# wyhuai/DDNM

Hardware: AMD Instinct MI355X
Metric: restored images/sec @256×256, 100 DDIM steps, 4×SR; 1/2/4/8 GPU (higher is better)
Workload: dtype f32 (3x3 convolutions: fp32 operands carried as hi + lo fp16 halves, three fp16 MFMA products per product, fp32 accumulate -- operand error 2^-22, measured closer to fp64 than the fp32 MFMA kernel; everything else fp32); 1 GPU; celeba_hq.yml SVD sr_bicubic 4x, sigma_y=0, eta=0.85, T_sampling=100, batch_size=8 per GPU (BASELINE configs[1]); global_batch=8, image=3x256x256, parallelism=dp1 (image sharding)

## Files before the change

ddnm_amd/_lib.py:

```python
import ctypes
import os
from ctypes import POINTER, Structure, c_char_p, c_float, c_int32, c_int64, c_uint32, c_void_p

_HERE = os.path.dirname(os.path.abspath(__file__))
LIB_PATH = os.path.join(_HERE, "libddnm_hip.so")

c_f32p = c_void_p


class ConvDesc(Structure):
    _fields_ = [
        ("src0", c_void_p), ("src1", c_void_p), ("weight", c_void_p), ("bias", c_void_p),
        ("badd", c_void_p), ("res", c_void_p), ("gn_scale", c_void_p), ("gn_shift", c_void_p),
        ("out", c_void_p),
        ("B", c_int32), ("Hin", c_int32), ("Win", c_int32),
        ("C0", c_int32), ("C1", c_int32), ("Cout", c_int32),
        ("ksize", c_int32), ("stride", c_int32), ("pad", c_int32),
        ("Ho", c_int32), ("Wo", c_int32),
        ("ups", c_int32), ("gn_silu", c_int32), ("out_nchw", c_int32),
        ("badd_stride", c_int32), ("tile", c_int32),
        ("workspace", c_void_p), ("workspace_floats", c_int64),
        ("res_ups", c_int32), ("src_f16", c_int32),
        ("stats_out", c_void_p),
        ("skip0", c_void_p), ("skip1", c_void_p), ("skip_weight", c_void_p),
# ... 70 lines not shown
                                    c_int32, c_void_p]),
    "ddnm_gn_finalize_tiles_f32": (c_int32, [c_void_p, c_int32, c_int32, c_void_p, c_int32, c_int32, c_void_p, c_void_p,
                                             c_int32, c_int32, c_int32, c_float, c_void_p, c_void_p, c_void_p, c_int32,
                                             c_void_p, c_void_p]),
    "ddnm_gn_finalize_tiles_amax_f32": (c_int32, [c_void_p, c_int32, c_int32, c_void_p, c_int32, c_int32, c_void_p, c_void_p,
                                                  c_int32, c_int32, c_int32, c_float, c_void_p, c_void_p, c_void_p, c_int32,
                                                  c_void_p, c_void_p, c_void_p]),
    "ddnm_amax_bound_f32": (c_int32, [c_void_p, c_int64, c_int32, c_void_p, c_int64, c_int32, c_void_p, c_int32, c_void_p]),
    "ddnm_conv3x3_f16_f32": (c_int32, [POINTER(ConvDesc), c_void_p]),
    "ddnm_conv3x3_f16_supported": (c_int32, [POINTER(ConvDesc)]),
    "ddnm_conv3x3_f16_workspace_floats": (c_int64, [POINTER(ConvDesc)]),
    "ddnm_conv3x3_f16_stats_tiles": (c_int32, [POINTER(ConvDesc)]),
    "ddnm_conv3x3_s16_f32": (c_int32, [POINTER(ConvDesc), c_void_p]),
    "ddnm_conv3x3_s16_supported": (c_int32, [POINTER(ConvDesc)]),
    "ddnm_conv3x3_s16_persistent": (c_int32, [POINTER(ConvDesc)]),
    "ddnm_conv3x3_s16_ups_subpixel_supported": (c_int32, [POINTER(ConvDesc)]),
    "ddnm_conv3x3_s16_workspace_floats": (c_int64, [POINTER(ConvDesc)]),
    "ddnm_conv3x3_s16_stats_tiles": (c_int32, [POINTER(ConvDesc)]),
    "ddnm_conv3x3_s16_act_scale": (c_float, []),
    "ddnm_conv_gather_s16_f32": (c_int32, [POINTER(ConvDesc), c_void_p]),
    "ddnm_conv_gather_s16_supported": (c_int32, [POINTER(ConvDesc)]),
    "ddnm_conv_gather_s16_workspace_floats": (c_int64, [POINTER(ConvDesc)]),
    "ddnm_conv_gather_s16_stats_tiles": (c_int32, [POINTER(ConvDesc)]),
    "ddnm_conv16": (c_int32, [POINTER(Conv16Desc), c_void_p]),
    "ddnm_conv16_supported": (c_int32, [POINTER(Conv16Desc)]),
    "ddnm_conv16_fuses_fin": (c_int32, [POINTER(Conv16Desc)]),
    "ddnm_conv16_workspace_floats": (c_int64, [POINTER(Conv16Desc)]),
    "ddnm_conv16_stats_tiles": (c_int32, [POINTER(Conv16Desc)]),
    "ddnm_gn_apply_h16": (c_int32, [c_void_p, c_void_p, c_void_p, c_void_p, c_void_p, c_int32, c_int32, c_int32, c_int32,
                                    c_int32, c_int32, c_int32, c_void_p]),
    "ddnm_im2col3x3_h16": (c_int32, [c_void_p, c_void_p, c_void_p, c_void_p, c_void_p, c_int32, c_int32, c_int32, c_int32,
                                     c_int32, c_int32, c_void_p]),
    "ddnm_nchw_to_nhwc_h16": (c_int32, [c_void_p, c_void_p, c_int32, c_int32, c_int32, c_int32, c_void_p]),
    "ddnm_gn_stats_h16": (c_int32, [c_void_p, c_void_p, c_int32, c_int32, c_int32, c_int32, c_void_p]),
    "ddnm_attn16_d64": (c_int32, [c_void_p, c_void_p, c_int32, c_int32, c_int32, c_void_p]),
    "ddnm_conv1x1_f16_f32": (c_int32, [POINTER(ConvDesc), c_void_p]),
    "ddnm_conv1x1_f16_supported": (c_int32, [POINTER(ConvDesc)]),
    "ddnm_conv1x1_f16_workspace_floats": (c_int64, [POINTER(ConvDesc)]),
    "ddnm_conv1x1_f16_stats_tiles": (c_int32, [POINTER(ConvDesc)]),
    "ddnm_gn_stats_f32": (c_int32, [c_void_p, c_void_p, c_int32, c_int32, c_int32, c_int32, c_int32, c_void_p,
                                    c_int32, c_void_p]),
    "ddnm_gn_nchunk": (c_int32, [c_int32, c_int32]),
    "ddnm_gn_finalize_f32": (c_int32, [c_void_p, c_int32, c_void_p, c_void_p, c_int32, c_int32, c_int32, c_int32,
                                       c_float, c_void_p, c_void_p, c_void_p, c_int32, c_void_p, c_void_p]),
    "ddnm_bgemm_f32": (c_int32, [POINTER(GemmDesc), c_void_p]),
    "ddnm_gn_bwd_f32": (c_int32, [c_void_p, c_void_p, c_int32, c_void_p, c_void_p, c_void_p, c_int32, c_void_p, c_int32,
# ... 154 lines not shown
```

ddnm_amd/build.py:

```python
import hashlib
import os
import shutil
import subprocess
import sys

HERE = os.path.dirname(os.path.abspath(__file__))
CSRC = os.path.join(HERE, "csrc")
LIB = os.path.join(HERE, "libddnm_hip.so")
STAMP = os.path.join(HERE, ".libddnm_hip.stamp")
OBJ = os.path.join(HERE, "_obj")
SOURCES = ["conv_igemm_f32.hip", "conv_igemm_f16.hip", "conv_s16_persist.hip", "conv_s16_subpixel.hip", "conv_gather_s16.hip", "conv_small_f32.hip", "conv1x1_f16.hip", "conv16.hip", "act16.hip", "attn16.hip", "attn_d512.hip", "attn16_bwd.hip", "gemm_f32.hip", "groupnorm.hip", "misc.hip", "ddnm_step.hip", "fwht.hip", "backward.hip", "metrics.hip"]
FLAGS = ["--offload-arch=gfx950", "-O3", "-std=c++17", "-fPIC", "-shared", "-Wall", "-Wno-unused-function"]


def _hipcc():
    for c in (os.environ.get("HIPCC"), shutil.which("hipcc"), "/opt/rocm/bin/hipcc"):
        if c and os.path.exists(c):
            return c
    raise RuntimeError("hipcc not found (set HIPCC)")


def _digest():
    h = hashlib.sha256()
    for f in sorted(os.listdir(CSRC)) + ["../../include/ddnm_hip.h"]:
        with open(os.path.join(CSRC, f), "rb") as fh:
            h.update(f.encode() + fh.read())
    h.update(" ".join(FLAGS).encode())
    return h.hexdigest()


LAST_BUILD = {"compiled": False}


def build(force=False, verbose=False):
# ... 64 lines not shown
```

ddnm_amd/csrc/conv_s16_persist.hip:

```cpp
#include <type_traits>

#include "conv_common.h"

typedef unsigned u32x4 __attribute__((ext_vector_type(4)));

namespace {
constexpr int P_WM = 4, P_WN = 2, P_MT = 2, P_NT = 2;
constexpr int P_NTHREADS = 512, P_BN = 128;
constexpr int P_LDH = 72, P_KCH = 32;
constexpr int P_MAXH = 340, P_HWD = 34;
constexpr int P_HCOLS = 8, P_HRPP = P_NTHREADS / P_HCOLS, P_HR = (P_MAXH + P_HRPP - 1) / P_HRPP, P_HSPLIT = (P_HR + 1) / 2;
constexpr int P_BR = P_BN / (P_NTHREADS / 8);
constexpr int P_NWB = 3, P_WTILE = P_BN * 128;
constexpr int P_HBYTES = 2 * P_MAXH * P_LDH * 2;
constexpr int P_NOUT = P_MT * P_NT * 16;
enum { K_MID = 0, K_LAST = 1, K_FIRST = 2 };

constexpr int p_spread(int tap) { return tap == 0 ? 10 : (tap <= 6 ? 9 : 0); }
constexpr int p_first_of(int tap) { return tap == 0 ? 0 : (tap <= 7 ? 10 + 9 * (tap - 1) : P_NOUT); }
static_assert(p_first_of(7) == P_NOUT, "64 values over taps 0..6");
constexpr int p_extra(int kind, int tap, bool has_res, bool ascale) {
    return kind == K_FIRST ? p_spread(tap) + (tap == 0 ? 1 : 0)
                           : (kind == K_LAST ? (tap == 0 ? 4 + (ascale ? 1 : 0) : 0) + (has_res ? p_spread(tap) : 0) : 0);
}
// ... 440 lines not shown
        if (!have_next) break;
        v = vn;
        cur_base = next_base;
        cur_stats = next_stats;
        epi_cur = epi_next;
        pending = true;
    }
    __syncthreads();
    store_stats();
#pragma unroll
    for (int k = 0; k < P_NOUT; ++k) __builtin_amdgcn_raw_buffer_store_b32(__float_as_uint(outv[k]), r_out, o_lane, o_soff(pend_base, k), 0);
}

bool conv3x3_s16_persist_eligible(const ConvArgs& p) {
    const ddnm_conv_desc& d = p.d;
    const long tiles = (long)p.m_tiles * p.n_tiles;
    if (d.skip0 && (!d.amax_in || d.res)) return false;
    return p.ksplit == 1 && tiles >= 512 && p.TW == 32 && !d.res_ups && !d.out_nchw && p.Cin / P_KCH >= 2 &&
           (int64_t)d.B * d.Ho * d.Wo * d.Cout * 4 < ((int64_t)1 << 31) && (int64_t)p.m_tiles * d.Cout * 8 < ((int64_t)1 << 31);
}

int conv3x3_s16_persist_launch(const ConvArgs& p, hipStream_t s) {
    const int cus = conv_persist_grid_cus();
    const int total = p.m_tiles * p.n_tiles;
    const dim3 grid(total < cus ? total : cus);
    const bool asc = p.d.amax_in != nullptr, res = p.d.res != nullptr;
    if (p.d.skip0) { DDNM_LAUNCH((conv3x3_s16_persist_kernel<true, false, true>), grid, dim3(P_NTHREADS), 0, s, p, total); }
    else if (asc && res) { DDNM_LAUNCH((conv3x3_s16_persist_kernel<true, true>), grid, dim3(P_NTHREADS), 0, s, p, total); }
    else if (asc) { DDNM_LAUNCH((conv3x3_s16_persist_kernel<true, false>), grid, dim3(P_NTHREADS), 0, s, p, total); }
    else if (res) { DDNM_LAUNCH((conv3x3_s16_persist_kernel<false, true>), grid, dim3(P_NTHREADS), 0, s, p, total); }
    else { DDNM_LAUNCH((conv3x3_s16_persist_kernel<false, false>), grid, dim3(P_NTHREADS), 0, s, p, total); }
    return 0;
}
```

ddnm_amd/csrc/conv_s16_subpixel.hip:

```cpp
#include <type_traits>

#include "conv_common.h"

typedef unsigned u32x4 __attribute__((ext_vector_type(4)));

namespace {
constexpr int Q_WM = 4, Q_WN = 2, Q_MT = 2, Q_NT = 2;
constexpr int Q_NTHREADS = 512, Q_BN = 128;
constexpr int Q_LDH = 72, Q_KCH = 32;
constexpr int Q_MAXH = 340, Q_HWD = 34;
constexpr int Q_HCOLS = 8, Q_HRPP = Q_NTHREADS / Q_HCOLS, Q_HR = (Q_MAXH + Q_HRPP - 1) / Q_HRPP;
constexpr int Q_BR = Q_BN / (Q_NTHREADS / 8);
constexpr int Q_NWB = 3, Q_WTILE = Q_BN * 128;
constexpr int Q_HBYTES = 2 * Q_MAXH * Q_LDH * 2;
constexpr int Q_NOUT = Q_MT * Q_NT * 16;
constexpr int Q_STEPS = 4;
enum { Q_MID = 0, Q_LAST = 1, Q_FIRST = 2 };

constexpr int q_first_of(int s) { return s == 0 ? 0 : (s == 1 ? 22 : (s == 2 ? 43 : Q_NOUT)); }
constexpr int q_extra(int kind, int s) {
    return (s == 0 ? Q_HR : 0) + (kind == Q_FIRST ? q_first_of(s + 1) - q_first_of(s) + (s == 0 ? 1 : 0) : (kind == Q_LAST && s == 0 ? 3 : 0));
}
constexpr int q_wait(int kind, int s) { return Q_BR + (s >= 1 ? q_extra(kind, s - 1) : q_extra(kind, 3)); }
static_assert(q_extra(Q_FIRST, 3) == 0 && q_extra(Q_MID, 3) == 0 && q_extra(Q_LAST, 3) == 0, "step 3 issues its weight tile only");
// ... 324 lines not shown
            c0 = 1;
        }
        for (int chunk = c0; chunk < nchunks - 1; ++chunk) run_chunk(ic<Q_MID>{}, chunk);
        run_last();
        finalize();
        if (!have_next) break;
        v += G;
        cur_base = next_base;
        cur_stats = next_stats;
        cur_py = next_py;
        epi_cur = epi_next;
        pending = true;
    }
    __syncthreads();
    store_stats();
#pragma unroll
    for (int k = 0; k < Q_NOUT; ++k) __builtin_amdgcn_raw_buffer_store_b32(__float_as_uint(outv[k]), r_out, o_lane, o_soff(pend_base, k), 0);
}

int conv_persist_grid_cus() {
    constexpr int MAXDEV = 64;
    static int cached[MAXDEV];
    int dev = 0;
    if (hipGetDevice(&dev) != hipSuccess || dev < 0 || dev >= MAXDEV) return 256;
    int cus = cached[dev];
    if (cus <= 0) {
        if (hipDeviceGetAttribute(&cus, hipDeviceAttributeMultiprocessorCount, dev) != hipSuccess || cus <= 0) cus = 256;
        cus -= cus % 8;
        if (cus <= 0) cus = 8;
        cached[dev] = cus;
    }
    return cus;
}

bool conv3x3_s16_ups_subpixel_ok(const ddnm_conv_desc* d) {
    if (!d || !d->ups || d->ksize != 3 || d->stride != 1 || d->pad != 1 || d->Ho != d->Hin || d->Wo != d->Win) return false;
    if (d->B <= 0 || d->Hin <= 0 || d->Win <= 0 || ((d->Hin | d->Win) & 1)) return false;
    const int hs = d->Hin / 2, ws = d->Win / 2, cin = d->C0 + d->C1;
    if (ws % 32 || hs % 8 || d->C0 <= 0 || d->C1 < 0 || cin % Q_KCH || d->C0 % Q_KCH || cin / Q_KCH < 2 || d->Cout <= 0 || d->Cout % 64) return false;
    if (d->src_f16 || d->out_nchw || d->res || d->res_ups || d->badd || d->gn_scale || d->skip0) return false;
    if (!conv_sizes_addressable(d)) return false;
    const int64_t lim = (int64_t)1 << 31;
    return (int64_t)d->B * d->Ho * d->Wo * d->Cout * 4 < lim && (int64_t)d->B * (d->Ho * d->Wo / 256) * d->Cout * 8 < lim &&
           (int64_t)4 * d->Cout * Q_STEPS * cin * 4 < lim && (int64_t)d->B * hs * ws / 256 * (d->Cout / 32) < lim;
}

int conv3x3_s16_ups_subpixel_run(const ddnm_conv_desc* d, hipStream_t s) {
    if (!d || !d->src0 || !d->weight || !d->out || !d->amax_in || !(d->acc_scale > 0.f)) return DDNM_E_BADARG;
    if (d->C1 > 0 && !d->src1) return DDNM_E_BADARG;
    if (!conv3x3_s16_ups_subpixel_ok(d)) return DDNM_E_SHAPE;
    ConvArgs p;
    p.d = *d;
    p.Cin = d->C0 + d->C1;
    p.ntaps = Q_STEPS;
    p.Hs = d->Hin / 2;
    p.Ws = d->Win / 2;
    p.m_tiles = d->B * (p.Hs * p.Ws / 256);
    p.n_tiles = d->Cout / 32;
    p.TW = 32;
    p.TW_log2 = 5;
    p.tiles_x = p.Ws / 32;
    p.ksplit = 1;
    p.ws = nullptr;
    const int total = p.m_tiles * p.n_tiles;
    const int cus = conv_persist_grid_cus();
    DDNM_LAUNCH(conv2x2x4_s16_subpixel_kernel, dim3(total < cus ? total : cus), dim3(Q_NTHREADS), 0, s, p, total);
    return 0;
}
```

ddnm_amd/guided_diffusion/models.py:

```python
import math
import os
from collections import OrderedDict

import torch

from .. import ops
from . import _net

GN_EPS = 1e-6
SPLIT16 = os.environ.get("DDNM_CONV_F32", "split16") != "mfma32"
UPS_SUBPIXEL = os.environ.get("DDNM_UPS_SUBPIXEL", "1")
UPS_SUBPIXEL_MIN_TILES = 128
CIN_PAD = 32


class _ResBlock:
    def __init__(self, name, cin, cout):
        self.name, self.cin, self.cout = name, cin, cout
        self.temb_off = None


class _Attn:
    def __init__(self, name, c):
        self.name, self.c = name, c


class Model(_net.GraphedNet):
    def __init__(self, config, device=None, split16=None):
        self.config = config
        self.split16 = SPLIT16 if split16 is None else bool(split16)
        self.ups_subpixel = UPS_SUBPIXEL if self.split16 else "0"
        self.fused_attn = self.split16
        self.fused_attn_max_tokens = 64
        m = config.model
        self.ch, self.out_ch, self.ch_mult = m.ch, m.out_ch, tuple(m.ch_mult)
        self.num_res_blocks = m.num_res_blocks
        self.attn_resolutions = list(m.attn_resolutions)
        self.in_channels = m.in_channels
        self.resolution = config.data.image_size
        self.temb_ch = 4 * self.ch
        self.num_resolutions = len(self.ch_mult)
        if not m.resamp_with_conv:
            raise NotImplementedError("resamp_with_conv=False is not on the DDNM hot path")
        self.device = torch.device("cuda") if device is None else torch.device(device)
        self._plan()
        self.w = None
        self._reset_host_state()

    def _plan(self):
        ch, mult, nrb = self.ch, self.ch_mult, self.num_res_blocks
        in_mult = (1,) + mult
        res = self.resolution
        self.down = []
        self.res_blocks = []
# ... 333 lines not shown
        t = t.to(device=x.device, dtype=torch.float32).contiguous()
        emb = ops.timestep_embedding(t, w["temb.freq"], order=0)
        temb = ops.linear(emb, w["temb.dense.0.weight"], w["temb.dense.0.bias"])
        temb = ops.linear(temb, w["temb.dense.1.weight"], w["temb.dense.1.bias"], silu_in=True)
        tproj = ops.linear(temb, w["temb_proj_cat.weight"], w["temb_proj_cat.bias"], silu_in=True)

        if "conv_in.weight.im2col" in w:
            xin = ops.nchw_im2col3x3_pad(x.contiguous(), CIN_PAD)
            hs = [ops.conv2d(xin, w["conv_in.weight.im2col"], self.ch, 1, bias=w["conv_in.bias"], emit_stats=True)]
        else:
            xin = ops.nchw_to_nhwc_pad(x.contiguous(), CIN_PAD)
            hs = [ops.conv2d(xin, w["conv_in.weight"], self.ch, 3, bias=w["conv_in.bias"], emit_stats=True)]
        for lvl, (blocks, attns, has_down, c) in enumerate(self.down):
            for ib, rb in enumerate(blocks):
                h = self._resblock(rb, hs[-1], None, tproj)
                if attns:
                    h = self._attn(attns[ib], h)
                hs.append(h)
            if has_down:
                n = f"down.{lvl}.downsample.conv"
                src = hs[-1]
                hs.append(ops.conv2d(src, w[n + ".weight"], c, 3, bias=w[n + ".bias"], stride=2, pad=0,
                                     out_hw=(src.t.shape[1] // 2, src.t.shape[2] // 2), emit_stats=True,
                                     weight_s16=w.get(n + ".s16")))
        h = hs[-1]
        h = self._resblock(self.mid[0], h, None, tproj)
        h = self._attn(self.mid[1], h)
        h = self._resblock(self.mid[2], h, None, tproj)
        for lvl in reversed(range(self.num_resolutions)):
            blocks, attns, has_up, c = self.up[lvl]
            for ib, rb in enumerate(blocks):
                h = self._resblock(rb, h, hs.pop(), tproj)
                if attns:
                    h = self._attn(attns[ib], h)
            if has_up:
                n = f"up.{lvl}.upsample.conv"
                if self._ups_subpixel(n, h.t.shape, c):
                    h = ops.conv2d(h, w[n + ".weight"], c, 3, bias=w[n + ".bias"], ups=True, emit_stats=True,
                                   weight_s16=w[n + ".s16_subpixel"], ups_subpixel=True)
                    continue
                h = ops.conv2d(h, w[n + ".weight"], c, 3, bias=w[n + ".bias"], ups=True, emit_stats=True,
                               weight_s16=w.get(n + ".s16"))
        gn = self._gn(h, None, "norm_out")
        return ops.conv2d(h, w["conv_out.weight"], self.out_ch, 3, gn=gn, gn_silu=True, bias=w["conv_out.bias"],
                          out_nchw=True)

    def _ups_subpixel(self, n, shape, c):
        if self.ups_subpixel == "0" or (n + ".s16_subpixel") not in self.w:
            return False
        B, H, W = shape[0], shape[1], shape[2]
        if self.ups_subpixel != "all" and B * (H * W // 256) * (c // 32) < UPS_SUBPIXEL_MIN_TILES:
            return False
        return ops.conv_runs_ups_subpixel(B, H, W, c, c)

    def __call__(self, x, t):
        return self.forward(x, t)
```

ddnm_amd/ops.py:

```python
import ctypes

import numpy as np
import torch

from . import _lib
from ._lib import Conv16Desc, ConvDesc, GemmDesc, StepScalars, check


def _p(t):
    return None if t is None else t.data_ptr()


def _stream():
    return torch.cuda.current_stream().cuda_stream


def _f32c(t, name):
    if t.dtype != torch.float32 or not t.is_contiguous() or not t.is_cuda:
        raise ValueError(f"{name}: expected a contiguous float32 device tensor, got {t.dtype} "
                         f"contiguous={t.is_contiguous()} device={t.device}")
    return t


class KernelTimer:
# ... 157 lines not shown


def upsample_weight_s16(w):
    sc = s16_weight_scale(upsample_phase_weights(w))
    return (pack_upsample_conv_weight_s16(w, sc), sc, None)


def conv_runs_ups_subpixel(B, H, W, cin, cout):
    d = _shape_desc(B, 2 * H, 2 * W, cin, cout)
    d.ups, d.flags = 1, UPS_SUBPIXEL
    return _lib.lib().ddnm_conv3x3_s16_ups_subpixel_supported(ctypes.byref(d)) == 1


def conv_runs_s16(B, H, W, cin, cout, ups=False):
    return _lib.lib().ddnm_conv3x3_s16_supported(ctypes.byref(_shape_desc(B, H, W, cin, cout))) == 1


def conv_runs_s16_gather(B, H, W, cin, cout, ksize=3, stride=1):
    if _NO_S16_GATHER:
        return False
    return _lib.lib().ddnm_conv_gather_s16_supported(ctypes.byref(_shape_desc(B, H, W, cin, cout, ksize, stride))) == 1


_S16_ACT_SCALE = None
_NO_S16_GATHER = False


def _s16_act_scale():
    global _S16_ACT_SCALE
    if _S16_ACT_SCALE is None:
        _S16_ACT_SCALE = float(_lib.lib().ddnm_conv3x3_s16_act_scale())
    return _S16_ACT_SCALE


def conv_runs_f16(B, H, W, cin, cout, ksize=3):
    L = _lib.lib()
    d = _shape_desc(B, H, W, cin, cout, ksize)
    return (L.ddnm_conv3x3_f16_supported if ksize == 3 else L.ddnm_conv1x1_f16_supported)(ctypes.byref(d)) == 1


_F16_PREPASS_MIN_COUT = 256
_f16_scratch_buf = {}


def _f16_scratch(device, numel, slot=0):
    key = (device, slot, _stream())
# ... 9 lines not shown


def amax_bound(a0, a1=None):
    def src(a):
        if a is None:
            return None, 0, 0
        if isinstance(a, Act) and a.stats is not None:
            B = a.t.shape[0]
            return a.stats, a.stats.numel() // B, 1
        t = tensor_of(a)
        return _f32c(t, "amax source"), t.numel() // t.shape[0], 0
    t0 = tensor_of(a0)
    B = t0.shape[0]
    p0, n0, k0 = src(a0)
    p1, n1, k1 = src(a1)
    out = torch.empty(B * AMAX_N, dtype=torch.float32, device=t0.device)
    check(_lib.lib().ddnm_amax_bound_f32(_p(p0), n0, k0, _p(p1), n1, k1, _p(out), B, _stream()), "ddnm_amax_bound_f32")
    return out


def conv2d(src0, weight, cout, ksize, *, src1=None, bias=None, badd=None, badd_stride=0, res=None, res_ups=False,
           gn=None, gn_silu=True, stride=1, pad=None, ups=False, out=None, out_nchw=False, out_hw=None, tile=0,
           emit_stats=False, weight_f16=None, skip=None, skip_weight=None, skip_weight_f16=None, weight_s16=None,
           raw_amax=None, one_tile=False, ups_subpixel=False):
    a_src0, a_src1 = src0, src1
    src0, src1, res = tensor_of(src0), tensor_of(src1), tensor_of(res)
    B, Hs, Ws, C0 = src0.shape
    C1 = 0 if src1 is None else src1.shape[3]
    Hin, Win = (2 * Hs, 2 * Ws) if ups else (Hs, Ws)
    if pad is None:
        pad = ksize // 2
    if out_hw is None:
        Ho, Wo = (Hin // stride, Win // stride)
    else:
        Ho, Wo = out_hw
    if out is None:
        shape = (B, cout, Ho, Wo) if out_nchw else (B, Ho, Wo, cout)
        out = torch.empty(shape, dtype=torch.float32, device=src0.device)
    d = ConvDesc()
    d.src0, d.src1, d.weight = _p(_f32c(src0, "src0")), _p(src1), _p(_f32c(weight, "weight"))
    d.bias, d.badd, d.res = _p(bias), _p(badd), _p(res)
    d.gn_scale, d.gn_shift = (None, None) if gn is None else (_p(gn[0]), _p(gn[1]))
    d.out = _p(out)
    d.B, d.Hin, d.Win, d.C0, d.C1, d.Cout = B, Hin, Win, C0, C1, cout
    d.ksize, d.stride, d.pad, d.Ho, d.Wo = ksize, stride, pad, Ho, Wo
    d.ups, d.gn_silu, d.out_nchw = int(ups), int(gn_silu), int(out_nchw)
    d.badd_stride, d.tile, d.res_ups = badd_stride, tile, int(res_ups)
    d.flags = 1 if (one_tile or FORCE_ONE_TILE) else 0
    L = _lib.lib()
    if ups_subpixel:
        d.flags = UPS_SUBPIXEL
        if (not ups or weight_s16 is None or weight_f16 is not None or skip is not None
                or L.ddnm_conv3x3_s16_ups_subpixel_supported(ctypes.byref(d)) != 1):
            raise ValueError(f"ups_subpixel: launch (B={B}, {Hs}x{Ws} -> {Ho}x{Wo}, Cin={C0 + C1}, Cout={cout}) does not "
                             "qualify (ddnm_conv3x3_s16_ups_subpixel_supported)")
    if out_nchw and cout <= 4 and skip is None and weight_f16 is None and L.ddnm_conv3x3_small_cout_f32_supported(ctypes.byref(d)) == 1:
        _launch(L.ddnm_conv3x3_small_cout_f32, d, "ddnm_conv3x3_small_cout_f32",
                lambda: ("conv3x3_small_cout_f32", 2.0 * B * Ho * Wo * cout * 9 * C0,
                         (B, Ho, Wo, C0, cout, 3, 1, 0, 0, gn is not None, False)))
        return Act(out, None, 0) if emit_stats else out
    f16, f16_1x1 = False, False
    if skip is not None:
        s0, s1 = tensor_of(skip[0]), tensor_of(skip[1])
        d.skip0, d.skip1 = _p(s0), _p(s1)
        d.SC0, d.SC1 = s0.shape[3], (0 if s1 is None else s1.shape[3])
    s16 = ups_subpixel or (weight_s16 is not None and weight_f16 is None and ksize == 3 and stride == 1
           and (skip is None or (weight_s16[2] is not None and gn is not None and d.SC0 % 32 == 0 and d.SC1 % 32 == 0))
           and L.ddnm_conv3x3_s16_supported(ctypes.byref(d)) == 1)
    s16g = (not s16 and weight_s16 is not None and weight_f16 is None and skip is None and not _NO_S16_GATHER
            and L.ddnm_conv_gather_s16_supported(ctypes.byref(d)) == 1)
    if s16 or s16g:
        d.weight = weight_s16[0].data_ptr()
        d.acc_scale = 1.0 / (float(weight_s16[1]) * _s16_act_scale())
        if gn is None or skip is not None:
            if raw_amax is None:
                raw_amax = amax_bound(*skip) if skip is not None else amax_bound(a_src0, a_src1)
            d.amax_in = raw_amax.data_ptr()
    if weight_f16 is not None:
        if ksize == 3:
            f16 = L.ddnm_conv3x3_f16_supported(ctypes.byref(d)) == 1
            if (not f16 and stride == 1 and not ups and skip is None and not out_nchw and not res_ups
                    and Hs * Ws < 256 and (C0 | C1) % 8 == 0):
                d.ksize, d.pad, d.C0, d.C1, d.gn_scale, d.gn_shift = 1, 0, 9 * (C0 + C1), 0, None, None
                if L.ddnm_conv1x1_f16_supported(ctypes.byref(d)) == 1:
                    col = _f16_scratch(src0.device, B * Hs * Ws * 9 * (C0 + C1), slot=1)
                    check(L.ddnm_im2col3x3_f16(_p(src0), _p(src1), None if gn is None else _p(gn[0]),
                                               None if gn is None else _p(gn[1]), col.data_ptr(), B, Hs, Ws, C0, C1,
                                               int(gn_silu), _stream()), "ddnm_im2col3x3_f16")
                    d.src0, d.src1, d.src_f16 = col.data_ptr(), None, 1
                    f16 = f16_1x1 = True
                    gn = None
                else:
                    d.ksize, d.pad, d.C0, d.C1 = 3, pad, C0, C1
                    d.gn_scale, d.gn_shift = (None, None) if gn is None else (_p(gn[0]), _p(gn[1]))
        elif ksize == 1 and skip is None:
            d.gn_scale, d.gn_shift = None, None
            f16 = f16_1x1 = L.ddnm_conv1x1_f16_supported(ctypes.byref(d)) == 1
            if not f16 and gn is not None:
                d.gn_scale, d.gn_shift = _p(gn[0]), _p(gn[1])
    if f16:
        d.weight = weight_f16.data_ptr()
        if gn is not None and (f16_1x1 or cout >= _F16_PREPASS_MIN_COUT):
            h16 = _f16_scratch(src0.device, B * Hs * Ws * (C0 + C1))
            check(L.ddnm_gn_apply_f16(_p(src0), _p(src1), _p(gn[0]), _p(gn[1]), h16.data_ptr(), B, Hs * Ws, C0, C1,
                                      int(gn_silu), _stream()), "ddnm_gn_apply_f16")
            d.src0, d.src1, d.C0, d.C1 = h16.data_ptr(), None, C0 + C1, 0
            d.gn_scale, d.gn_shift, d.src_f16 = None, None, 1
    if skip is not None:
        d.skip_weight = _p(skip_weight_f16) if f16 else (weight_s16[2].data_ptr() if s16 else _p(skip_weight))
        if f16 and skip_weight_f16 is None:
            raise ValueError("fp16 launch with a fused shortcut needs skip_weight_f16")
    if f16_1x1:
        fn_run, fn_tiles, fn_ws = L.ddnm_conv1x1_f16_f32, L.ddnm_conv1x1_f16_stats_tiles, L.ddnm_conv1x1_f16_workspace_floats
    elif f16:
        fn_run, fn_tiles, fn_ws = L.ddnm_conv3x3_f16_f32, L.ddnm_conv3x3_f16_stats_tiles, L.ddnm_conv3x3_f16_workspace_floats
    elif s16:
        fn_run, fn_tiles, fn_ws = L.ddnm_conv3x3_s16_f32, L.ddnm_conv3x3_s16_stats_tiles, L.ddnm_conv3x3_s16_workspace_floats
    elif s16g:
        fn_run, fn_tiles, fn_ws = (L.ddnm_conv_gather_s16_f32, L.ddnm_conv_gather_s16_stats_tiles,
                                   L.ddnm_conv_gather_s16_workspace_floats)
    else:
        fn_run, fn_tiles, fn_ws = L.ddnm_conv2d_f32, L.ddnm_conv2d_f32_stats_tiles, L.ddnm_conv2d_f32_workspace_floats
    stats, tiles = None, 0
    if emit_stats and not _NO_FUSED_GN:
        tiles = fn_tiles(ctypes.byref(d))
        if tiles > 0:
            stats = torch.empty(B * tiles * cout * 2, dtype=torch.float32, device=src0.device)
            d.stats_out = stats.data_ptr()
    need = fn_ws(ctypes.byref(d))
    if need > 0:
        ws = _conv_workspace(src0.device, need)
        d.workspace, d.workspace_floats = ws.data_ptr(), ws.numel()

    def record():
        if f16_1x1:
            variant = "conv1x1_f16<256x128>"
        elif f16:
            variant = "conv3x3_halo_f16<256x128>"
        elif s16:
            variant = ("conv2x2x4_s16_subpixel<256x128>" if ups_subpixel else
                       "conv3x3_s16_persist<256x128>" if L.ddnm_conv3x3_s16_persistent(ctypes.byref(d)) == 1 else "conv3x3_halo_s16<256x128>")
        elif s16g:
            variant = "conv_gather_s16"
        else:
            tn = L.ddnm_conv2d_f32_tile_n(ctypes.byref(d))
            kind = "conv3x3_halo_f32" if (ksize == 3 and stride == 1) else "conv_gather_f32"
            variant = kind + {128: "<128x128>", 64: "<64x64>", 32: "<128x32>"}[tn]
        flops = 2.0 * B * Ho * Wo * cout * (ksize * ksize * (C0 + C1) + d.SC0 + d.SC1)
        if ups_subpixel:
            flops *= 16.0 / 36.0
        return variant, flops, (B, Ho, Wo, C0 + C1, cout, ksize, stride, int(ups), d.SC0 + d.SC1, gn is not None,
                                res is not None)
    _launch(fn_run, d, "ddnm_conv2d", record)
    if _S16_CHECK and (s16 or s16g) and not bool(torch.isfinite(out).all()):
        raise FloatingPointError(f"split-fp16 launch produced non-finite values (B={B}, {Hin}x{Win}, Cin={C0 + C1}, "
                                 f"Cout={cout}, k={ksize}): an operand left fp16 range; DDNM_CONV_F32=mfma32 selects the "
                                 "all-fp32 engine")
    if emit_stats:
        return Act(out, stats, tiles)
    return out


CONV16_COUT_ALIGN = 256


def _f16c(t, name):
    if t.dtype != torch.float16 or not t.is_contiguous() or not t.is_cuda:
        raise ValueError(f"{name}: expected a contiguous float16 device tensor, got {t.dtype} "
                         f"contiguous={t.is_contiguous()} device={t.device}")
    return t


def pack_conv_weight16(w, cin_pad=None):
    if w.dim() == 2:
        w = w[:, :, None, None]
    cout, cin, kh, kw = w.shape
    cin_pad = cin if cin_pad is None else cin_pad
# ... 516 lines not shown
```

include/ddnm_hip.h:

```cpp
#ifndef DDNM_HIP_H
#define DDNM_HIP_H

#include <stdint.h>

#ifdef __cplusplus
extern "C" {
#endif

#define DDNM_E_BADARG (-1)
#define DDNM_E_SHAPE (-2)

int ddnm_version(void);
const char* ddnm_build_digest(void);
int ddnm_sizeof(int which);
const char* ddnm_error_string(int code);

typedef struct ddnm_conv_desc {
    const float* src0;
    const float* src1;
    const float* weight;
    const float* bias;
    const float* badd;
    const float* res;
    const float* gn_scale;
// ... 36 lines not shown
int ddnm_conv2d_f32_fuses_skip(const ddnm_conv_desc* d);

int ddnm_conv3x3_small_cout_f32(const ddnm_conv_desc* d, void* stream);
int ddnm_conv3x3_small_cout_f32_supported(const ddnm_conv_desc* d);

int ddnm_conv3x3_f16_f32(const ddnm_conv_desc* d, void* stream);
int ddnm_conv3x3_f16_supported(const ddnm_conv_desc* d);
int64_t ddnm_conv3x3_f16_workspace_floats(const ddnm_conv_desc* d);
int ddnm_conv3x3_f16_stats_tiles(const ddnm_conv_desc* d);

int ddnm_conv3x3_s16_f32(const ddnm_conv_desc* d, void* stream);
int ddnm_conv3x3_s16_supported(const ddnm_conv_desc* d);
int ddnm_conv3x3_s16_persistent(const ddnm_conv_desc* d);
int64_t ddnm_conv3x3_s16_workspace_floats(const ddnm_conv_desc* d);
int ddnm_conv3x3_s16_stats_tiles(const ddnm_conv_desc* d);
int ddnm_conv3x3_s16_ups_subpixel_supported(const ddnm_conv_desc* d);
float ddnm_conv3x3_s16_act_scale(void);

int ddnm_conv_gather_s16_f32(const ddnm_conv_desc* d, void* stream);
int ddnm_conv_gather_s16_supported(const ddnm_conv_desc* d);
int64_t ddnm_conv_gather_s16_workspace_floats(const ddnm_conv_desc* d);
int ddnm_conv_gather_s16_stats_tiles(const ddnm_conv_desc* d);

int ddnm_conv1x1_f16_f32(const ddnm_conv_desc* d, void* stream);
int ddnm_conv1x1_f16_supported(const ddnm_conv_desc* d);
int64_t ddnm_conv1x1_f16_workspace_floats(const ddnm_conv_desc* d);
int ddnm_conv1x1_f16_stats_tiles(const ddnm_conv_desc* d);

typedef struct ddnm_conv16_desc {
    const void* src;
    const void* weight;
    const float* bias;
    const void* res;
    const void* skip0;
    const void* skip1;
    const void* skip_weight;
    void* out;
    float* stats_out;
    float* workspace;
    int64_t workspace_floats;
    int32_t B, H, W;
    int32_t Cin, Cout;
    int32_t ksize;
    int32_t ups, res_ups;
    int32_t SC0, SC1;
    const void* src1;
// ... 260 lines not shown
```

Measured before the change: 6.312 images/sec.

## Add halo-patch split-fp16 kernel for stride-2 downsample convolutions

Adds a dedicated split-fp16 MFMA kernel for 3x3 stride-2, pad-0 downsample convolutions. For each 128-pixel output tile it stages a de-interleaved input patch in LDS once per channel chunk and reuses it across all nine taps, instead of going through the generic gather kernel. Weights stream through a triple buffer, and the patch prefetch is spread across taps. It is enabled by default, but the model gates it to layers with exactly 256 output tiles, so only a small part of the network is affected. The persistent-grid CU query also now fails with an error instead of assuming 256 CUs.

```diff
diff --git a/ddnm_amd/_lib.py b/ddnm_amd/_lib.py
--- a/ddnm_amd/_lib.py
+++ b/ddnm_amd/_lib.py
@@ -116,6 +116,10 @@
     "ddnm_conv_gather_s16_supported": (c_int32, [POINTER(ConvDesc)]),
     "ddnm_conv_gather_s16_workspace_floats": (c_int64, [POINTER(ConvDesc)]),
     "ddnm_conv_gather_s16_stats_tiles": (c_int32, [POINTER(ConvDesc)]),
+    "ddnm_conv_s16_down_f32": (c_int32, [POINTER(ConvDesc), c_void_p]),
+    "ddnm_conv_s16_down_supported": (c_int32, [POINTER(ConvDesc)]),
+    "ddnm_conv_s16_down_workspace_floats": (c_int64, [POINTER(ConvDesc)]),
+    "ddnm_conv_s16_down_stats_tiles": (c_int32, [POINTER(ConvDesc)]),
     "ddnm_conv16": (c_int32, [POINTER(Conv16Desc), c_void_p]),
     "ddnm_conv16_supported": (c_int32, [POINTER(Conv16Desc)]),
     "ddnm_conv16_fuses_fin": (c_int32, [POINTER(Conv16Desc)]),
diff --git a/ddnm_amd/build.py b/ddnm_amd/build.py
--- a/ddnm_amd/build.py
+++ b/ddnm_amd/build.py
@@ -9,7 +9,7 @@
 LIB = os.path.join(HERE, "libddnm_hip.so")
 STAMP = os.path.join(HERE, ".libddnm_hip.stamp")
 OBJ = os.path.join(HERE, "_obj")
-SOURCES = ["conv_igemm_f32.hip", "conv_igemm_f16.hip", "conv_s16_persist.hip", "conv_s16_subpixel.hip", "conv_gather_s16.hip", "conv_small_f32.hip", "conv1x1_f16.hip", "conv16.hip", "act16.hip", "attn16.hip", "attn_d512.hip", "attn16_bwd.hip", "gemm_f32.hip", "groupnorm.hip", "misc.hip", "ddnm_step.hip", "fwht.hip", "backward.hip", "metrics.hip"]
+SOURCES = ["conv_igemm_f32.hip", "conv_igemm_f16.hip", "conv_s16_persist.hip", "conv_s16_subpixel.hip", "conv_s16_down.hip", "conv_gather_s16.hip", "conv_small_f32.hip", "conv1x1_f16.hip", "conv16.hip", "act16.hip", "attn16.hip", "attn_d512.hip", "attn16_bwd.hip", "gemm_f32.hip", "groupnorm.hip", "misc.hip", "ddnm_step.hip", "fwht.hip", "backward.hip", "metrics.hip"]
 FLAGS = ["--offload-arch=gfx950", "-O3", "-std=c++17", "-fPIC", "-shared", "-Wall", "-Wno-unused-function"]
 
 
diff --git a/ddnm_amd/csrc/conv_s16_down.hip b/ddnm_amd/csrc/conv_s16_down.hip
--- /dev/null
+++ b/ddnm_amd/csrc/conv_s16_down.hip
@@ -0,0 +1,267 @@
+#include <type_traits>
+
+#include "conv_common.h"
+
+namespace {
+constexpr int DS_KC = 32;
+constexpr int DS_LDH = 72;
+constexpr int DS_BM = 128, DS_BN = 128;
+constexpr int DS_AR = 19;
+constexpr int DS_ROWS = 32 * DS_AR;
+constexpr int DS_BR = DS_BN / 32;
+constexpr int DS_NWB = 3, DS_WTILE = DS_BN * 128;
+constexpr int DS_TAPS = 9;
+constexpr int ds_part(int t) { return t <= 5 ? 3 * t : (t == 6 ? 17 : DS_AR); }
+static_assert(ds_part(0) == 0 && ds_part(7) == DS_AR && ds_part(DS_TAPS) == DS_AR, "taps 7 and 8 request weights only");
+constexpr int ds_wait(int t) { return DS_BR + (t >= 1 ? ds_part(t) - ds_part(t - 1) : 0); }
+
+template <int V>
+using ic = std::integral_constant<int, V>;
+}
+
+template <int TWl>
+__global__ __launch_bounds__(256) void conv3x3_s16_down_kernel(const ConvArgs p) {
+    constexpr int WM = 2, WN = 2, MT = 2, NT = 2, BM = DS_BM, BN = DS_BN, AR = DS_AR, BR = DS_BR, LDH = DS_LDH;
+    constexpr int NWB = DS_NWB, WTILE = DS_WTILE;
+    __shared__ __attribute__((aligned(1024))) char lds_all[NWB * WTILE + DS_ROWS * LDH * 2];
+    char* const Bs = lds_all;
+    _Float16* const Ps = reinterpret_cast<_Float16*>(lds_all + NWB * WTILE);
+
+    const ddnm_conv_desc& d = p.d;
+    const int tid = threadIdx.x, lane = tid & 63;
+    const int wave = __builtin_amdgcn_readfirstlane(tid >> 6);
+    const int wm = wave / WN, wn = wave % WN;
+    const int tile_id = xcd_swizzle(blockIdx.x, gridDim.x);
+    const int n_tile = tile_id % p.n_tiles, m_tile = tile_id / p.n_tiles;
+    const int slice = blockIdx.y;
+    const TileMap tm = make_tilemap<BM>(p, m_tile);
+    const int img = tm.img;
+    constexpr int TW = 1 << TWl, TH = BM >> TWl;
+    constexpr int PW = 2 * TW + 1, PR = (2 * TH + 1) * PW;
+    static_assert(PR <= DS_ROWS, "the patch fits its buffer");
+    float ascale, inv_ascale;
+    s16_operand_scale(d.amax_in, img, false, ascale, inv_ascale);
+    float epi_scale = d.acc_scale * inv_ascale;
+    int e_ntile = n_tile, e_mtile = m_tile, e_ty0 = tm.ty0, e_tx0 = tm.tx0, e_img = img;
+    asm volatile("" : "+v"(epi_scale), "+v"(e_ntile), "+v"(e_mtile), "+v"(e_ty0), "+v"(e_tx0), "+v"(e_img));
+
+    const int lrow = lane >> 3, lpiece = lane & 7;
+    const int wswz = (((wave & 1) << 2) | (lrow >> 1));
+    const unsigned w_rowlen = (unsigned)DS_TAPS * (unsigned)p.Cin * 4u;
+    const __amdgpu_buffer_rsrc_t r_w = __builtin_amdgcn_make_buffer_rsrc(
+        const_cast<void*>(reinterpret_cast<const void*>(d.weight)), 0, (unsigned)d.Cout * w_rowlen, 0x00020000);
+    const unsigned w_voff = (unsigned)(n_tile * BN + wave * 8 + lrow) * w_rowlen + (unsigned)((lpiece ^ wswz) * 16);
+    auto issue_w = [&](int chunk, int tap, int buf) {
+        char* dst = Bs + buf * WTILE + wave * 1024;
+        const unsigned so = ((unsigned)tap * p.Cin + (unsigned)chunk * DS_KC) * 4u;
+#pragma unroll
+        for (int j = 0; j < BR; ++j)
+            __builtin_amdgcn_raw_ptr_buffer_load_lds(r_w, (__attribute__((address_space(3))) void*)(dst + j * 4096), 16, w_voff,
+                                                     so + (unsigned)j * 32u * w_rowlen, 0, 0);
+    };
+
+    constexpr unsigned AOOB = 0x80000000u;
+    const __amdgpu_buffer_rsrc_t r_s = __builtin_amdgcn_make_buffer_rsrc(
+        const_cast<float*>(d.src0), 0, (unsigned)d.B * d.Hin * d.Win * d.C0 * 4u, 0x00020000);
+    const int c4 = tid & 7, row0 = tid >> 3;
+    unsigned a_vo[AR];
+#pragma unroll
+    for (int i = 0; i < AR; ++i) {
+        const int s = row0 + 32 * i;
+        const int py = s / PW, q = s - py * PW;
+        const int iy = 2 * tm.ty0 + py, ix = 2 * tm.tx0 + (q <= TW ? 2 * q : 2 * (q - TW) - 1);
+        const bool ok = s < PR && iy < d.Hin && ix < d.Win;
+        a_vo[i] = ok ? ((unsigned)((img * d.Hin + iy) * d.Win + ix) * (unsigned)d.C0 + c4 * 4) * 4u : AOOB;
+    }
+    f32x4 a_st[AR];
+    auto prefetch_patch = [&](int chunk, bool live, int i0, int i1) {
+#pragma unroll
+        for (int i = 0; i < AR; ++i)
+            if (i >= i0 && i < i1) a_st[i] = __builtin_bit_cast(f32x4, __builtin_amdgcn_raw_buffer_load_b128(r_s, live ? a_vo[i] : AOOB, (unsigned)chunk * DS_KC * 4u, 0));
+    };
+    auto stage_patch = [&]() {
+#pragma unroll
+        for (int i = 0; i < AR; ++i) split_store(&Ps[(row0 + 32 * i) * LDH + c4 * 4], a_st[i], ascale);
+    };
+
+    f32x16 acc[MT][NT];
+#pragma unroll
+    for (int i = 0; i < MT; ++i)
+#pragma unroll
+        for (int j = 0; j < NT; ++j)
+#pragma unroll
+            for (int r = 0; r < 16; ++r) acc[i][j][r] = 0.f;
+    int a_off[MT];
+#pragma unroll
+    for (int i = 0; i < MT; ++i) {
+        const int m = (wm * MT + i) * 32 + (lane & 31);
+        a_off[i] = (2 * (m >> TWl) * PW + (m & (TW - 1))) * LDH + (lane >> 5) * 8;
+    }
+    const int b_frag = ((wn * NT * 32 + (lane & 31)) * 128) + ((((lane >> 5) ^ (((lane & 31) >> 1) & 7))) << 4);
+
+    auto mfma_step = [&](int ky, int kx, int buf) {
+        const int step_off = (ky * PW + (kx == 1 ? TW + 1 : 0) + (kx == 2 ? 1 : 0)) * LDH;
+        const char* bf = Bs + buf * WTILE;
+#pragma unroll
+        for (int ks = 0; ks < 2; ++ks) {
+            half8 ah[MT], al[MT], bh[NT], bl[NT];
+#pragma unroll
+            for (int i = 0; i < MT; ++i) {
+                ah[i] = *reinterpret_cast<const half8*>(Ps + a_off[i] + step_off + ks * 16);
+                al[i] = *reinterpret_cast<const half8*>(Ps + a_off[i] + step_off + ks * 16 + 32);
+            }
+#pragma unroll
+            for (int j = 0; j < NT; ++j) {
+                bh[j] = *reinterpret_cast<const half8*>(bf + ((b_frag ^ (ks << 5)) + j * 32 * 128));
+                bl[j] = *reinterpret_cast<const half8*>(bf + ((b_frag ^ ((ks + 2) << 5)) + j * 32 * 128));
+            }
+#pragma unroll
+            for (int i = 0; i < MT; ++i)
+#pragma unroll
+                for (int j = 0; j < NT; ++j) acc[i][j] = __builtin_amdgcn_mfma_f32_32x32x16_f16(al[i], bh[j], acc[i][j], 0, 0, 0);
+#pragma unroll
+            for (int i = 0; i < MT; ++i)
+#pragma unroll
+                for (int j = 0; j < NT; ++j) acc[i][j] = __builtin_amdgcn_mfma_f32_32x32x16_f16(ah[i], bl[j], acc[i][j], 0, 0, 0);
+#pragma unroll
+            for (int i = 0; i < MT; ++i)
+#pragma unroll
+                for (int j = 0; j < NT; ++j) acc[i][j] = __builtin_amdgcn_mfma_f32_32x32x16_f16(ah[i], bh[j], acc[i][j], 0, 0, 0);
+        }
+    };
+
+    const int nchunks = p.Cin / DS_KC;
+    const int c_begin = nchunks * slice / p.ksplit, c_end = nchunks * (slice + 1) / p.ksplit;
+    prefetch_patch(c_begin, true, 0, AR);
+    asm volatile("" ::: "memory");
+    __builtin_amdgcn_sched_barrier(0);
+    issue_w(c_begin, 0, 0);
+    issue_w(c_begin, 1, 1);
+    asm volatile("" ::: "memory");
+    __builtin_amdgcn_sched_barrier(0);
+    stage_patch();
+
+    int wb = 0;
+    auto step_body = [&](auto TAP, int chunk) {
+        constexpr int tap = decltype(TAP)::value;
+        asm volatile("s_waitcnt vmcnt(%0) lgkmcnt(0)" ::"n"(ds_wait(tap)) : "memory");
+        __builtin_amdgcn_s_barrier();
+        asm volatile("" ::: "memory");
+        if constexpr (ds_part(tap) < ds_part(tap + 1)) {
+            prefetch_patch(chunk + 1, chunk + 1 < c_end, ds_part(tap), ds_part(tap + 1));
+            asm volatile("" ::: "memory");
+            __builtin_amdgcn_sched_barrier(0);
+        }
+        int nc = tap + 2 < DS_TAPS ? chunk : chunk + 1, nt = (tap + 2) % DS_TAPS;
+        if (nc >= c_end) { nc = c_end - 1; nt = DS_TAPS - 1; }
+        issue_w(nc, nt, wb == 0 ? NWB - 1 : wb - 1);
+        asm volatile("" ::: "memory");
+        __builtin_amdgcn_sched_barrier(0);
+        mfma_step(tap / 3, tap % 3, wb);
+        wb = wb == NWB - 1 ? 0 : wb + 1;
+    };
+    for (int chunk = c_begin; chunk < c_end; ++chunk) {
+        step_body(ic<0>{}, chunk);
+        step_body(ic<1>{}, chunk);
+        step_body(ic<2>{}, chunk);
+        step_body(ic<3>{}, chunk);
+        step_body(ic<4>{}, chunk);
+        step_body(ic<5>{}, chunk);
+        step_body(ic<6>{}, chunk);
+        step_body(ic<7>{}, chunk);
+        step_body(ic<8>{}, chunk);
+        if (chunk + 1 < c_end) {
+            asm volatile("s_waitcnt lgkmcnt(0)" ::: "memory");
+            __builtin_amdgcn_s_barrier();
+            asm volatile("" ::: "memory");
+            stage_patch();
+        }
+    }
+    asm volatile("s_waitcnt vmcnt(0)" ::: "memory");
+    __syncthreads();
+    TileMap te = tm;
+    te.img = __builtin_amdgcn_readfirstlane(e_img);
+    te.ty0 = __builtin_amdgcn_readfirstlane(e_ty0);
+    te.tx0 = __builtin_amdgcn_readfirstlane(e_tx0);
+    conv_epilogue<WM, WN, MT, NT>(p, te, __builtin_amdgcn_readfirstlane(e_ntile), __builtin_amdgcn_readfirstlane(e_mtile), slice, acc,
+                                  reinterpret_cast<float*>(Ps), epi_scale);
+}
+
+static int down_tile_w(const ddnm_conv_desc* d) {
+    if (!d || d->ksize != 3 || d->stride != 2 || d->pad != 0 || d->C1 != 0 || d->ups || d->res_ups) return 0;
+    if (d->B <= 0 || d->Hin <= 0 || d->Win <= 0 || d->Ho <= 0 || d->Wo <= 0) return 0;
+    if (d->Ho != d->Hin / 2 || d->Wo != d->Win / 2 || ((d->Hin | d->Win) & 1)) return 0;
+    if (d->C0 <= 0 || d->C0 % DS_KC || d->Cout <= 0 || d->Cout % DS_BN) return 0;
+    if (d->gn_scale || d->gn_shift || d->skip0 || d->skip1 || d->src1 || d->out_nchw || d->src_f16 || d->res || d->badd) return 0;
+    if (d->flags & DDNM_CONV_UPS_SUBPIXEL) return 0;
+    if (!conv_sizes_addressable(d)) return 0;
+    {
+        if ((int64_t)d->B * d->Hin * d->Win * d->C0 * 4 >= (int64_t)1 << 31) return 0;
+    }
+    int tw = 0;
+    if (d->Wo % 32 == 0 && d->Ho % 4 == 0) tw = 32;
+    else if (d->Wo % 16 == 0 && d->Ho % 8 == 0) tw = 16;
+    return tw;
+}
+
+static int plan_down(const ddnm_conv_desc* d) {
+    const int nchunks = d->C0 / DS_KC;
+    long tiles = (long)d->B * (d->Ho * d->Wo / DS_BM) * (d->Cout / DS_BN);
+    if (tiles * nchunks < 256) tiles *= 4;
+    int ks = 1;
+    if (tiles < 192) {
+        ks = (int)((512 + tiles - 1) / tiles);
+        if (ks > nchunks) ks = nchunks;
+        if (ks > 16) ks = 16;
+        if (ks < 1) ks = 1;
+    }
+    return ks;
+}
+
+extern "C" int ddnm_conv_s16_down_supported(const ddnm_conv_desc* d) { return down_tile_w(d) > 0 ? 1 : 0; }
+
+extern "C" int64_t ddnm_conv_s16_down_workspace_floats(const ddnm_conv_desc* d) {
+    if (down_tile_w(d) <= 0) return DDNM_E_SHAPE;
+    const int ks = plan_down(d);
+    return ks > 1 ? (int64_t)ks * d->B * d->Ho * d->Wo * d->Cout : 0;
+}
+
+extern "C" int ddnm_conv_s16_down_stats_tiles(const ddnm_conv_desc* d) {
+    if (down_tile_w(d) <= 0) return DDNM_E_SHAPE;
+    return plan_down(d) > 1 ? splitk_stats_tiles(d) : d->Ho * d->Wo / DS_BM;
+}
+
+extern "C" int ddnm_conv_s16_down_f32(const ddnm_conv_desc* d, void* stream) {
+    if (!d || !d->src0 || !d->weight || !d->out) return DDNM_E_BADARG;
+    if (!d->amax_in) return DDNM_E_BADARG;
+    if (!(d->acc_scale > 0.f)) return DDNM_E_BADARG;
+    const int tw = down_tile_w(d);
+    if (tw <= 0) return DDNM_E_SHAPE;
+    int ks = plan_down(d);
+    if (ks > 1) {
+        const int64_t need = (int64_t)ks * d->B * d->Ho * d->Wo * d->Cout;
+        if (!d->workspace || d->workspace_floats < need) {
+            if (d->stats_out) return DDNM_E_BADARG;
+            ks = 1;
+        }
+    }
+    ConvArgs p;
+    p.d = *d;
+    p.Cin = d->C0;
+    p.ntaps = DS_TAPS;
+    p.Hs = d->Hin;
+    p.Ws = d->Win;
+    p.m_tiles = d->B * (d->Ho * d->Wo / DS_BM);
+    p.n_tiles = d->Cout / DS_BN;
+    p.TW = tw;
+    p.TW_log2 = tw == 32 ? 5 : 4;
+    p.tiles_x = d->Wo / tw;
+    p.ksplit = ks;
+    p.ws = d->workspace;
+    hipStream_t s = (hipStream_t)stream;
+    const dim3 grid(p.m_tiles * p.n_tiles, ks);
+    if (tw == 32) { DDNM_LAUNCH(conv3x3_s16_down_kernel<5>, grid, dim3(256), 0, s, p); }
+    else { DDNM_LAUNCH(conv3x3_s16_down_kernel<4>, grid, dim3(256), 0, s, p); }
+    if (ks > 1) return launch_splitk_reduce(p, s);
+    return 0;
+}
diff --git a/ddnm_amd/csrc/conv_s16_persist.hip b/ddnm_amd/csrc/conv_s16_persist.hip
--- a/ddnm_amd/csrc/conv_s16_persist.hip
+++ b/ddnm_amd/csrc/conv_s16_persist.hip
@@ -486,6 +486,7 @@
 
 int conv3x3_s16_persist_launch(const ConvArgs& p, hipStream_t s) {
     const int cus = conv_persist_grid_cus();
+    if (cus <= 0) return DDNM_E_BADARG;
     const int total = p.m_tiles * p.n_tiles;
     const dim3 grid(total < cus ? total : cus);
     const bool asc = p.d.amax_in != nullptr, res = p.d.res != nullptr;
diff --git a/ddnm_amd/csrc/conv_s16_subpixel.hip b/ddnm_amd/csrc/conv_s16_subpixel.hip
--- a/ddnm_amd/csrc/conv_s16_subpixel.hip
+++ b/ddnm_amd/csrc/conv_s16_subpixel.hip
@@ -370,10 +370,10 @@
     constexpr int MAXDEV = 64;
     static int cached[MAXDEV];
     int dev = 0;
-    if (hipGetDevice(&dev) != hipSuccess || dev < 0 || dev >= MAXDEV) return 256;
+    if (hipGetDevice(&dev) != hipSuccess || dev < 0 || dev >= MAXDEV) return -1;
     int cus = cached[dev];
     if (cus <= 0) {
-        if (hipDeviceGetAttribute(&cus, hipDeviceAttributeMultiprocessorCount, dev) != hipSuccess || cus <= 0) cus = 256;
+        if (hipDeviceGetAttribute(&cus, hipDeviceAttributeMultiprocessorCount, dev) != hipSuccess || cus <= 0) return -1;
         cus -= cus % 8;
         if (cus <= 0) cus = 8;
         cached[dev] = cus;
@@ -412,6 +412,7 @@
     p.ws = nullptr;
     const int total = p.m_tiles * p.n_tiles;
     const int cus = conv_persist_grid_cus();
+    if (cus <= 0) return DDNM_E_BADARG;
     DDNM_LAUNCH(conv2x2x4_s16_subpixel_kernel, dim3(total < cus ? total : cus), dim3(Q_NTHREADS), 0, s, p, total);
     return 0;
 }
diff --git a/ddnm_amd/guided_diffusion/models.py b/ddnm_amd/guided_diffusion/models.py
--- a/ddnm_amd/guided_diffusion/models.py
+++ b/ddnm_amd/guided_diffusion/models.py
@@ -11,6 +11,9 @@
 SPLIT16 = os.environ.get("DDNM_CONV_F32", "split16") != "mfma32"
 UPS_SUBPIXEL = os.environ.get("DDNM_UPS_SUBPIXEL", "1")
 UPS_SUBPIXEL_MIN_TILES = 128
+DOWN_HALO = os.environ.get("DDNM_DOWN_HALO", "1")
+DOWN_HALO_MIN_TILES = 256
+DOWN_HALO_MAX_TILES = 256
 CIN_PAD = 32
 
 
@@ -30,6 +33,7 @@
         self.config = config
         self.split16 = SPLIT16 if split16 is None else bool(split16)
         self.ups_subpixel = UPS_SUBPIXEL if self.split16 else "0"
+        self.down_halo = DOWN_HALO if self.split16 else "0"
         self.fused_attn = self.split16
         self.fused_attn_max_tokens = 64
         m = config.model
@@ -409,7 +413,7 @@
                 src = hs[-1]
                 hs.append(ops.conv2d(src, w[n + ".weight"], c, 3, bias=w[n + ".bias"], stride=2, pad=0,
                                      out_hw=(src.t.shape[1] // 2, src.t.shape[2] // 2), emit_stats=True,
-                                     weight_s16=w.get(n + ".s16")))
+                                     weight_s16=w.get(n + ".s16"), down_halo=self._down_halo(n, src.t.shape, c)))
         h = hs[-1]
         h = self._resblock(self.mid[0], h, None, tproj)
         h = self._attn(self.mid[1], h)
@@ -432,6 +436,15 @@
         return ops.conv2d(h, w["conv_out.weight"], self.out_ch, 3, gn=gn, gn_silu=True, bias=w["conv_out.bias"],
                           out_nchw=True)
 
+    def _down_halo(self, n, shape, c):
+        if self.down_halo == "0" or (n + ".s16") not in self.w:
+            return False
+        B, H, W = shape[0], shape[1], shape[2]
+        tiles = B * ((H // 2) * (W // 2) // ops.DOWN_TILE) * (c // 128)
+        if self.down_halo != "all" and not DOWN_HALO_MIN_TILES <= tiles <= DOWN_HALO_MAX_TILES:
+            return False
+        return ops.conv_runs_s16_down(B, H, W, c, c)
+
     def _ups_subpixel(self, n, shape, c):
         if self.ups_subpixel == "0" or (n + ".s16_subpixel") not in self.w:
             return False
diff --git a/ddnm_amd/ops.py b/ddnm_amd/ops.py
--- a/ddnm_amd/ops.py
+++ b/ddnm_amd/ops.py
@@ -203,6 +203,11 @@
     return _lib.lib().ddnm_conv_gather_s16_supported(ctypes.byref(_shape_desc(B, H, W, cin, cout, ksize, stride))) == 1
 
 
+def conv_runs_s16_down(B, H, W, cin, cout):
+    return _lib.lib().ddnm_conv_s16_down_supported(ctypes.byref(_shape_desc(B, H, W, cin, cout, 3, 2))) == 1
+
+
+DOWN_TILE = 128
 _S16_ACT_SCALE = None
 _NO_S16_GATHER = False
 
@@ -258,7 +263,7 @@
 def conv2d(src0, weight, cout, ksize, *, src1=None, bias=None, badd=None, badd_stride=0, res=None, res_ups=False,
            gn=None, gn_silu=True, stride=1, pad=None, ups=False, out=None, out_nchw=False, out_hw=None, tile=0,
            emit_stats=False, weight_f16=None, skip=None, skip_weight=None, skip_weight_f16=None, weight_s16=None,
-           raw_amax=None, one_tile=False, ups_subpixel=False):
+           raw_amax=None, one_tile=False, ups_subpixel=False, down_halo=False):
     a_src0, a_src1 = src0, src1
     src0, src1, res = tensor_of(src0), tensor_of(src1), tensor_of(res)
     B, Hs, Ws, C0 = src0.shape
@@ -303,9 +308,16 @@
     s16 = ups_subpixel or (weight_s16 is not None and weight_f16 is None and ksize == 3 and stride == 1
            and (skip is None or (weight_s16[2] is not None and gn is not None and d.SC0 % 32 == 0 and d.SC1 % 32 == 0))
            and L.ddnm_conv3x3_s16_supported(ctypes.byref(d)) == 1)
-    s16g = (not s16 and weight_s16 is not None and weight_f16 is None and skip is None and not _NO_S16_GATHER
+    s16d = False
+    if down_halo:
+        s16d = (not s16 and weight_s16 is not None and weight_f16 is None and skip is None and gn is None and src1 is None
+                and res is None and badd is None and L.ddnm_conv_s16_down_supported(ctypes.byref(d)) == 1)
+        if not s16d:
+            raise ValueError(f"down_halo: launch (B={B}, {Hin}x{Win} -> {Ho}x{Wo}, Cin={C0 + C1}, Cout={cout}, k={ksize}, "
+                             f"stride={stride}, pad={pad}) does not qualify (ddnm_conv_s16_down_supported)")
+    s16g = (not s16 and not s16d and weight_s16 is not None and weight_f16 is None and skip is None and not _NO_S16_GATHER
             and L.ddnm_conv_gather_s16_supported(ctypes.byref(d)) == 1)
-    if s16 or s16g:
+    if s16 or s16g or s16d:
         d.weight = weight_s16[0].data_ptr()
         d.acc_scale = 1.0 / (float(weight_s16[1]) * _s16_act_scale())
         if gn is None or skip is not None:
@@ -352,6 +364,8 @@
         fn_run, fn_tiles, fn_ws = L.ddnm_conv3x3_f16_f32, L.ddnm_conv3x3_f16_stats_tiles, L.ddnm_conv3x3_f16_workspace_floats
     elif s16:
         fn_run, fn_tiles, fn_ws = L.ddnm_conv3x3_s16_f32, L.ddnm_conv3x3_s16_stats_tiles, L.ddnm_conv3x3_s16_workspace_floats
+    elif s16d:
+        fn_run, fn_tiles, fn_ws = L.ddnm_conv_s16_down_f32, L.ddnm_conv_s16_down_stats_tiles, L.ddnm_conv_s16_down_workspace_floats
     elif s16g:
         fn_run, fn_tiles, fn_ws = (L.ddnm_conv_gather_s16_f32, L.ddnm_conv_gather_s16_stats_tiles,
                                    L.ddnm_conv_gather_s16_workspace_floats)
@@ -376,6 +390,8 @@
         elif s16:
             variant = ("conv2x2x4_s16_subpixel<256x128>" if ups_subpixel else
                        "conv3x3_s16_persist<256x128>" if L.ddnm_conv3x3_s16_persistent(ctypes.byref(d)) == 1 else "conv3x3_halo_s16<256x128>")
+        elif s16d:
+            variant = "conv3x3_s16_down<128x128>"
         elif s16g:
             variant = "conv_gather_s16"
         else:
@@ -388,7 +404,7 @@
         return variant, flops, (B, Ho, Wo, C0 + C1, cout, ksize, stride, int(ups), d.SC0 + d.SC1, gn is not None,
                                 res is not None)
     _launch(fn_run, d, "ddnm_conv2d", record)
-    if _S16_CHECK and (s16 or s16g) and not bool(torch.isfinite(out).all()):
+    if _S16_CHECK and (s16 or s16g or s16d) and not bool(torch.isfinite(out).all()):
         raise FloatingPointError(f"split-fp16 launch produced non-finite values (B={B}, {Hin}x{Win}, Cin={C0 + C1}, "
                                  f"Cout={cout}, k={ksize}): an operand left fp16 range; DDNM_CONV_F32=mfma32 selects the "
                                  "all-fp32 engine")
diff --git a/include/ddnm_hip.h b/include/ddnm_hip.h
--- a/include/ddnm_hip.h
+++ b/include/ddnm_hip.h
@@ -82,6 +82,11 @@
 int64_t ddnm_conv_gather_s16_workspace_floats(const ddnm_conv_desc* d);
 int ddnm_conv_gather_s16_stats_tiles(const ddnm_conv_desc* d);
 
+int ddnm_conv_s16_down_f32(const ddnm_conv_desc* d, void* stream);
+int ddnm_conv_s16_down_supported(const ddnm_conv_desc* d);
+int64_t ddnm_conv_s16_down_workspace_floats(const ddnm_conv_desc* d);
+int ddnm_conv_s16_down_stats_tiles(const ddnm_conv_desc* d);
+
 int ddnm_conv1x1_f16_f32(const ddnm_conv_desc* d, void* stream);
 int ddnm_conv1x1_f16_supported(const ddnm_conv_desc* d);
 int64_t ddnm_conv1x1_f16_workspace_floats(const ddnm_conv_desc* d);
```

After: 6.300 images/sec. Within noise of the previous version (-0.2%).
